# wg-perception/PartsBasedDetector

Measured on AMD Instinct MI355X. Metric: detect() frames/sec, 640x480, 26-part person model, higher is better.
Workload: dtype f32

## Files before the change

### partsbaseddetector_amd/csrc/k_conv_split32.hpp

```cpp
typedef __bf16 bf16x8 __attribute__((ext_vector_type(8)));
typedef _Float16 f16x8 __attribute__((ext_vector_type(8)));
typedef unsigned u32x4 __attribute__((ext_vector_type(4)));
typedef float f32x4 __attribute__((ext_vector_type(4)));
typedef float f32x16 __attribute__((ext_vector_type(16)));

template <int NT, int NW, int PIN, int NS = 3, bool MIX = false>
__global__ __launch_bounds__(64 * NW) __attribute__((amdgpu_waves_per_eu(1, PIN ? 1 : 2))) void k_conv_split32(const ConvTile* __restrict__ tiles, const LevelDev* __restrict__ levels,
                                                             const uint16_t* __restrict__ feat, const uint16_t* __restrict__ filt,
                                                             float* __restrict__ resp, int nf, int ntl_bank, int ntile0, int ngroups,
                                                             int ntiles_total, int kh, int kw, const float* __restrict__ oscale) {
  extern __shared__ __attribute__((aligned(16))) char smem[];
  constexpr int ROWS = 4 * NW, NHALVES = 16 / ROWS, NTHR = 64 * NW, PPC = 4 * NS;
  const int TW = 16 + kw - 1, TH = ROWS + kh - 1, NC = TW * TH, PLANE = NC * 64;
  const int R = NHALVES * ngroups;
  const int lin = blockIdx.x;
  const int grp = lin / (8 * R), rem = lin - grp * (8 * R);
  const int tile_i = grp * 8 + (rem & 7), role = rem >> 3;
  if (tile_i >= ntiles_total) return;
  const int half = role & (NHALVES - 1), ngroup = role / NHALVES;
  const ConvTile t = tiles[tile_i];
  const LevelDev lv = levels[t.level];
  const int H = lv.ch, W = lv.cw;
  const int ty0 = t.y0 + ROWS * half, tx0 = t.x0;
  if (ty0 >= H) return;
  const int tid = threadIdx.x, lane = tid & 63, wave = __builtin_amdgcn_readfirstlane(tid >> 6);
  const uint16_t* F = feat + lv.cell_off * (NS * PBD_FLEN);
  {
    const int NPC = NC * PPC, oy = ty0 - kh / 2, ox = tx0 - kw / 2;
    constexpr unsigned ONE = NS == 3 ? 0x3F800000u : 0x6C000000u;
    auto cell_of = [](int i) { return NS == 3 ? (int)(((unsigned)i * 43691u) >> 19) : i >> 3; };
    const unsigned magic_tw = 0xFFFFFFFFu / (unsigned)TW + 1u;
    constexpr int BATCH = 12;
    for (int i0 = 0; i0 < NPC; i0 += NTHR * BATCH) {
      u32x4 v[BATCH];
#pragma unroll
      for (int j = 0; j < BATCH; ++j) {
        const int i = min(i0 + j * NTHR + tid, NPC - 1);
        const int cell = cell_of(i), piece = i - cell * PPC;
        const int cy = (int)__umulhi((unsigned)cell, magic_tw), cx = cell - cy * TW;
        const int y = min(max(oy + cy, 0), H - 1), x = min(max(ox + cx, 0), W - 1);
        v[j] = *(const u32x4*)(F + ((size_t)(y * W + x) * (NS * PBD_FLEN) + piece * 8));
      }
#pragma unroll
      for (int j = 0; j < BATCH; ++j) {
        const int i = i0 + j * NTHR + tid;
        if (i < NPC) {
          const int cell = cell_of(i), piece = i - cell * PPC;
          const int cy = (int)__umulhi((unsigned)cell, magic_tw), cx = cell - cy * TW;
          const int y = oy + cy, x = ox + cx;
          const bool inside = y >= 0 && y < H && x >= 0 && x < W;
          const u32x4 border = u32x4{0u, 0u, 0u, piece == 3 ? ONE : 0u};
          const int q = piece & 3;
          *(u32x4*)(smem + (piece >> 2) * PLANE + cell * 64 + ((q ^ ((cell >> 2) & 3)) << 4)) = inside ? v[j] : border;
        }
      }
    }
  }
  __syncthreads();
  const int col = lane & 15, kb = lane >> 4;
  const bool inner = col >= 4 && col < 12;
  const int kk = inner ? col - 4 : col < 4 ? col : col - 8;
  const int pos = ((kk >> 1) << 2) + (inner ? 0 : 2) + (kk & 1);
  const int vw = min(16, W - tx0), vh = min(ROWS, H - ty0), ncell = vw * vh;
  const int nmt = (ncell + 15) >> 4;
  const int mvalid = __builtin_amdgcn_readfirstlane(max(0, min(4, (nmt - wave + NW - 1) / NW)));
  const unsigned vw_magic = 65535u / (unsigned)vw + 1u;
  int cl0[4], cofs[4];
  bool cval[4];
#pragma unroll
  for (int m = 0; m < 4; ++m) {
    const int idx = 16 * (wave + NW * m) + pos;
    cval[m] = idx < ncell;
    const int ic = min(idx, ncell - 1);
    const int cy = (int)(((unsigned)ic * vw_magic) >> 16), cx = ic - cy * vw;
    cl0[m] = cy * TW + cx;
    cofs[m] = (ty0 + cy) * W + tx0 + cx;
  }
  const int ntb = ntile0 + ngroup * NT;
  const size_t bs_split = (size_t)ntl_bank * 512, bs_kstep = NS * bs_split, bs_tap = 2 * bs_kstep;
  const uint16_t* bl = filt + (size_t)ntb * 512 + (size_t)(kb >> 1) * bs_kstep + (kb & 1) * 256 + col * 8;
#ifdef PBD_BANK_PRIO
  __builtin_amdgcn_s_setprio(PBD_BANK_PRIO);
#endif

  constexpr int NTRI = NS == 3 ? 2 : 1;
  auto mfma3 = [](int tri, f32x4& d, const u32x4 (&fb)[NS], const u32x4 (&fa)[NS]) __attribute__((always_inline)) {
    if constexpr (NS == 3) {
      if (tri == 0)
        asm volatile("v_mfma_f32_16x16x32_bf16 %0, %1, %2, %0\n\tv_mfma_f32_16x16x32_bf16 %0, %3, %4, %0\n\tv_mfma_f32_16x16x32_bf16 %0, %5, %6, %0"
                     : "+a"(d) : "v"(fb[1]), "v"(fa[1]), "v"(fb[2]), "v"(fa[0]), "v"(fb[0]), "v"(fa[2]));
      else
        asm volatile("v_mfma_f32_16x16x32_bf16 %0, %1, %2, %0\n\tv_mfma_f32_16x16x32_bf16 %0, %3, %4, %0\n\tv_mfma_f32_16x16x32_bf16 %0, %3, %2, %0"
                     : "+a"(d) : "v"(fb[1]), "v"(fa[0]), "v"(fb[0]), "v"(fa[1]));
    } else {
      asm volatile("v_mfma_f32_16x16x32_f16 %0, %1, %2, %0\n\tv_mfma_f32_16x16x32_f16 %0, %3, %4, %0\n\tv_mfma_f32_16x16x32_f16 %0, %3, %2, %0"
                   : "+a"(d) : "v"(fb[1]), "v"(fa[0]), "v"(fb[0]), "v"(fa[1]));
    }
  };

  auto k_loop = [&](auto mv_tag) __attribute__((always_inline)) {
    constexpr int MV = decltype(mv_tag)::value, NU = 2 * MV * NTRI, NLD = 2 * NS, LPT = (NLD + NU - 2) / (NU - 1);
    static_assert(NU >= 2 && LPT * (NU - 1) >= NLD, "a step's statements carry the next step's filter loads");
    u32x4 a[4][NS], b[2][2][NS];
    f32x4 acc[2 * NT][MV];
#pragma unroll
    for (int ft = 0; ft < 2 * NT; ++ft)
// ... 24 lines not shown
          for (int m = 0; m < MV; ++m) {
#pragma unroll
            for (int q = 0; q < NTRI; ++q) {
              const int u = (h * MV + m) * NTRI + q;
              mfma3(q + 2 - NTRI, acc[2 * nt + h][m], b[slot][h], a[m]);
              if (u * LPT < NLD) {
                __builtin_amdgcn_sched_barrier(0);
#pragma unroll
                for (int k = u * LPT; k < (u + 1) * LPT && k < NLD; ++k)
                  b[slot ^ 1][k / NS][k % NS] = *(const u32x4*)(pl + (k % NS) * bs_split + (k / NS) * 128);
                __builtin_amdgcn_sched_barrier(0);
              }
            }
            if (last && h == 1) {
              __builtin_amdgcn_sched_barrier(0);
              ld_a(m, nextofs);
              __builtin_amdgcn_sched_barrier(0);
            }
          }
      }
    };
    const int ntap = kh * kw;
#pragma unroll
    for (int k = 0; k < NLD; ++k) b[0][k / NS][k % NS] = *(const u32x4*)(bl + (k % NS) * bs_split + (k / NS) * 128);
#pragma unroll
    for (int m = 0; m < MV; ++m) ld_a(m, 0);
    pad_acc();
    int ti = 0, tj = 0;
    const uint16_t* pt = bl;
    auto one_tap = [&](auto p_tag, int tap) __attribute__((always_inline)) {
      if (++tj == kw) { tj = 0; ++ti; }
      const bool more = tap + 1 < ntap;
      const uint16_t* pn = more ? pt + bs_tap : pt;
      tap_body(p_tag, pt, pn, more ? ti * TW + tj : 0);
      pt = pn;
    };
#pragma unroll 1
    for (int tap = 0; tap < ntap; tap += 1 + (NT & 1)) {
      one_tap(std::integral_constant<int, 0>(), tap);
      if constexpr (NT & 1) {
        if (tap + 1 >= ntap) break;
        one_tap(std::integral_constant<int, 1>(), tap + 1);
      }
    }
    pad_acc();

    float* Rl = resp + lv.cell_off * nf;
    const size_t HW = (size_t)H * W;
    int nfw = nf;
    if constexpr (MIX) { Rl += (size_t)(t.pad & 0xFFFF) * HW; nfw = t.pad >> 16; }
#pragma unroll
    for (int m = 0; m < MV; ++m) {
      if (cval[m]) {
#pragma unroll
        for (int ft = 0; ft < 2 * NT; ++ft) {
          const int f0 = 32 * ntb + 16 * ft + 4 * kb;
          float* pl = Rl + (size_t)f0 * HW + cofs[m];
#pragma unroll
          for (int r = 0; r < 4; ++r)
            if (f0 + r < nfw) pl[(size_t)r * HW] = NS == 3 ? acc[ft][m][r] : acc[ft][m][r] * oscale[f0 + r];
        }
      }
    }
  };
  switch (mvalid) {
    case 4: k_loop(std::integral_constant<int, 4>()); break;
    case 3: k_loop(std::integral_constant<int, 3>()); break;
    case 2: k_loop(std::integral_constant<int, 2>()); break;
    case 1: k_loop(std::integral_constant<int, 1>()); break;
    default: return;
  }
}

template <int NT, int NW, int PIN, int NS = 3, bool MIX = false>
static void launch_conv_split_t(const ConvTile* tiles, int ntiles, const LevelDev* levels, const uint16_t* feat_split, const uint16_t* wS,
                                float* resp, int nf, int ntl_bank, int ntile0, int ngroups, int kh, int kw, hipStream_t s, const float* oscale = nullptr,
                                int nf_stride = 0) {
  constexpr int ROWS = 4 * NW, NHALVES = 16 / ROWS;
  const size_t lds = (size_t)(16 + kw - 1) * (ROWS + kh - 1) * 64 * NS;
  static LdsOptIn optin;
  optin.ensure((const void*)k_conv_split32<NT, NW, PIN, NS, MIX>, lds);
  const int grid = (ntiles + 7) / 8 * 8 * NHALVES * ngroups;
  hipLaunchKernelGGL((k_conv_split32<NT, NW, PIN, NS, MIX>), dim3(grid), dim3(64 * NW), lds, s, tiles, levels, feat_split, wS, resp, MIX ? nf_stride : nf,
                     ntl_bank, ntile0, ngroups, ntiles, kh, kw, oscale);
}
template <int NW, int PIN, int NS, bool MIX = false>
static void launch_conv_split_groups(const ConvTile* tiles, int ntiles, const LevelDev* levels, const uint16_t* feat_split, const uint16_t* wS,
                                     float* resp, int nf, int kh, int kw, const float* oscale, hipStream_t s, int nf_stride = 0, int G = 5) {
  const int ntl = conv_split_ntiles(nf), full = ntl / G, rest = ntl - G * full;
  auto go = [&](int nt, int ntile0, int ngroups) {
    switch (nt) {
      case 1: launch_conv_split_t<1, NW, PIN, NS, MIX>(tiles, ntiles, levels, feat_split, wS, resp, nf, ntl, ntile0, ngroups, kh, kw, s, oscale, nf_stride); break;
      case 2: launch_conv_split_t<2, NW, PIN, NS, MIX>(tiles, ntiles, levels, feat_split, wS, resp, nf, ntl, ntile0, ngroups, kh, kw, s, oscale, nf_stride); break;
      case 3: launch_conv_split_t<3, NW, PIN, NS, MIX>(tiles, ntiles, levels, feat_split, wS, resp, nf, ntl, ntile0, ngroups, kh, kw, s, oscale, nf_stride); break;
      case 4: launch_conv_split_t<4, NW, PIN, NS, MIX>(tiles, ntiles, levels, feat_split, wS, resp, nf, ntl, ntile0, ngroups, kh, kw, s, oscale, nf_stride); break;
      case 5: launch_conv_split_t<5, NW, PIN, NS, MIX>(tiles, ntiles, levels, feat_split, wS, resp, nf, ntl, ntile0, ngroups, kh, kw, s, oscale, nf_stride); break;
      default: break;
    }
  };
  if (full) go(G, 0, full);
  if (rest) go(rest, G * full, 1);
}
```

### partsbaseddetector_amd/csrc/k_pyramid.hip

```cpp
#include <algorithm>
#include "pbd_internal.hpp"

typedef __attribute__((aligned(1))) unsigned u32_unaligned;

__device__ __forceinline__ int sat_short_dev(float v) {
  int i = __float2int_rn(v);
  return i < -32768 ? -32768 : (i > 32767 ? 32767 : i);
}

#define RPX 4
__global__ __launch_bounds__(256) void k_resize_linear_u8(const PyrJob* __restrict__ jobs, int cn, int sstride,
                                                          const uint8_t* __restrict__ src0, uint8_t* __restrict__ pyr) {
  const PyrJob a = jobs[blockIdx.y];
  const int dw = a.dw, dh = a.dh, sw = a.sw, sh = a.sh;
  const uint8_t* src = src0 + a.soff;
  uint8_t* dst = pyr + a.doff;
  const bool copy = (dw == sw && dh == sh);
  if (copy) {
    const int rowb = dw * cn, wpr = (rowb + 3) >> 2, nw = wpr * dh;
    for (int i = blockIdx.x * blockDim.x + threadIdx.x; i < nw; i += gridDim.x * blockDim.x) {
      const int y = i / wpr, k = i - y * wpr;
      const uint8_t* s = src + (size_t)y * sstride + 4 * k;
      uint8_t* d = dst + (size_t)y * rowb + 4 * k;
      if (4 * k + 4 <= rowb) *(u32_unaligned*)d = *(const u32_unaligned*)s;
      else for (int b = 0; 4 * k + b < rowb; ++b) d[b] = s[b];
    }
    return;
  }
  const double scale_x = 1. / ((double)dw / sw), scale_y = 1. / ((double)dh / sh);
  const int gpr = (dw + RPX - 1) / RPX, ngrp = gpr * dh;
  for (int i = blockIdx.x * blockDim.x + threadIdx.x; i < ngrp; i += gridDim.x * blockDim.x) {
    const int dy = i / gpr, gx = i - dy * gpr;
    float fy = (float)((dy + 0.5) * scale_y - 0.5);
    int sy = (int)floorf(fy);
    fy -= sy;
    const int b0 = sat_short_dev((1.f - fy) * 2048), b1 = sat_short_dev(fy * 2048);
    const int sy0 = sy < 0 ? 0 : (sy >= sh ? sh - 1 : sy);
    const int sy1 = sy + 1 < 0 ? 0 : (sy + 1 >= sh ? sh - 1 : sy + 1);
    const uint8_t* R0 = src + (size_t)sy0 * sstride;
    const uint8_t* R1 = src + (size_t)sy1 * sstride;
    uint8_t ob[RPX * 3];
    const int npx = min(RPX, dw - gx * RPX);
#pragma unroll
    for (int p = 0; p < RPX; ++p) {
      const int dx = min(gx * RPX + p, dw - 1);
      float fx = (float)((dx + 0.5) * scale_x - 0.5);
      int sx = (int)floorf(fx);
      fx -= sx;
      if (sx < 0) { fx = 0; sx = 0; }
      const bool edge = (sx + 1 >= sw);
      if (sx >= sw - 1) { fx = 0; sx = sw - 1; }
      const int a0 = sat_short_dev((1.f - fx) * 2048), a1 = sat_short_dev(fx * 2048);
      const uint8_t* S0 = R0 + sx * cn;
      const uint8_t* S1 = R1 + sx * cn;
      uint8_t p0[6], p1[6];
      if (cn == 3 && !edge) {
        const unsigned w00 = *(const u32_unaligned*)S0, w01 = *(const unsigned short __attribute__((aligned(1)))*)(S0 + 4);
        const unsigned w10 = *(const u32_unaligned*)S1, w11 = *(const unsigned short __attribute__((aligned(1)))*)(S1 + 4);
#pragma unroll
        for (int b = 0; b < 4; ++b) { p0[b] = (uint8_t)(w00 >> (8 * b)); p1[b] = (uint8_t)(w10 >> (8 * b)); }
        p0[4] = (uint8_t)w01; p0[5] = (uint8_t)(w01 >> 8); p1[4] = (uint8_t)w11; p1[5] = (uint8_t)(w11 >> 8);
      } else {
#pragma unroll
        for (int b = 0; b < 6; ++b) {
          const int o = (b < cn || !edge) && b < 2 * cn ? b : 0;
          p0[b] = S0[o]; p1[b] = S1[o];
        }
      }
#pragma unroll
      for (int c = 0; c < 3; ++c) {
        if (c < cn) {
          int r0, r1;
          if (edge) { r0 = p0[c] * 2048; r1 = p1[c] * 2048; }
          else { r0 = p0[c] * a0 + p0[c + cn] * a1; r1 = p1[c] * a0 + p1[c + cn] * a1; }
          const int v = (((b0 * (r0 >> 4)) >> 16) + ((b1 * (r1 >> 4)) >> 16) + 2) >> 2;
          ob[p * 3 + c] = (uint8_t)(v < 0 ? 0 : (v > 255 ? 255 : v));
        }
      }
    }
    uint8_t* d = dst + ((size_t)dy * dw + gx * RPX) * cn;
    if (cn == 3 && npx == RPX) {
#pragma unroll
      for (int k = 0; k < 3; ++k)
        *(u32_unaligned*)(d + 4 * k) = (unsigned)ob[4 * k] | ((unsigned)ob[4 * k + 1] << 8) | ((unsigned)ob[4 * k + 2] << 16) | ((unsigned)ob[4 * k + 3] << 24);
    } else {
      for (int p = 0; p < npx; ++p)
        for (int c = 0; c < cn; ++c) d[p * cn + c] = ob[p * 3 + c];
    }
  }
}

__device__ __forceinline__ int reflect101_dev(int p, int len) {
  if (len == 1) return 0;
  while ((unsigned)p >= (unsigned)len) p = p < 0 ? -p : 2 * len - 2 - p;
  return p;
}

#define PD_TW 32
#define PD_TH 8
#define PD_SW (2 * PD_TW + 3)
#define PD_SH (2 * PD_TH + 3)
template <int CN>
__global__ __launch_bounds__(256) void k_pyrdown_u8(const PyrJob* __restrict__ jobs, uint8_t* __restrict__ pyr) {
  constexpr int cn = CN;
  __shared__ __attribute__((aligned(4))) uint8_t tile[PD_SH][(PD_SW * CN + 3) & ~3];
  __shared__ unsigned short hs[PD_SH][PD_TW * CN];
  const PyrJob a = jobs[blockIdx.z];
  const int sw = a.sw, sh = a.sh;
  const int dw = (sw + 1) / 2, dh = (sh + 1) / 2;
  const int x0 = blockIdx.x * PD_TW, y0 = blockIdx.y * PD_TH;
  if (x0 >= dw || y0 >= dh) return;
  const uint8_t* src = pyr + a.soff;
  uint8_t* dst = pyr + a.doff;
  const int tid = threadIdx.x;
  const int sx0 = 2 * x0 - 2, sy0 = 2 * y0 - 2;
  const int rowb = PD_SW * cn, srow = sw * cn;
  {
    const int wpr = (rowb + 3) >> 2, nw = wpr * PD_SH;
    const bool xin = sx0 >= 0 && sx0 + PD_SW <= sw;
    for (int i = tid; i < nw; i += 256) {
      const int r = i / wpr, k = i - r * wpr;
      const uint8_t* srow_p = src + (size_t)reflect101_dev(sy0 + r, sh) * srow;
      unsigned v;
      if (xin && sx0 * cn + 4 * k + 4 <= srow) {
        v = *(const u32_unaligned*)(srow_p + sx0 * cn + 4 * k);
      } else {
        v = 0;
#pragma unroll
        for (int b = 0; b < 4; ++b) {
          const int cb = 4 * k + b;
          const int px = cb / cn, ch = cb - px * cn;
          const int sx = reflect101_dev(sx0 + min(px, PD_SW - 1), sw);
          v |= (unsigned)srow_p[sx * cn + ch] << (8 * b);
        }
      }
      *(unsigned*)&tile[r][4 * k] = v;
    }
  }
  __syncthreads();
  {
    const int n = PD_SH * PD_TW * cn;
    for (int i = tid; i < n; i += 256) {
      const int r = i / (PD_TW * cn), xc = i - r * (PD_TW * cn);
      const int x = xc / cn, c = xc - x * cn;
      const uint8_t* p = &tile[r][2 * x * cn + c];
      hs[r][xc] = (unsigned short)(p[0] + 4 * p[cn] + 6 * p[2 * cn] + 4 * p[3 * cn] + p[4 * cn]);
    }
  }
  __syncthreads();
  {
    const int n = PD_TH * PD_TW * cn;
    for (int i = tid; i < n; i += 256) {
      const int y = i / (PD_TW * cn), xc = i - y * (PD_TW * cn);
      const int x = xc / cn;
      if (y0 + y < dh && x0 + x < dw) {
        const int s = hs[2 * y][xc] + 4 * hs[2 * y + 1][xc] + 6 * hs[2 * y + 2][xc] + 4 * hs[2 * y + 3][xc] + hs[2 * y + 4][xc];
        dst[((size_t)(y0 + y) * dw + x0) * cn + xc] = (uint8_t)((s + 128) >> 8);
      }
    }
  }
}

void launch_resize(const PyrJob* jobs, int njobs, int maxpix, int cn, int sstride, const uint8_t* src, uint8_t* pyr, hipStream_t s) {
  if (njobs <= 0) return;
  dim3 grid((maxpix / RPX + 255) / 256 + 1, njobs);
  hipLaunchKernelGGL(k_resize_linear_u8, grid, dim3(256), 0, s, jobs, cn, sstride, src, pyr);
}

void launch_pyrdown(const PyrJob* jobs, int njobs, int maxw, int maxh, int cn, uint8_t* pyr, hipStream_t s) {
  if (njobs <= 0) return;
  dim3 grid((maxw + PD_TW - 1) / PD_TW, (maxh + PD_TH - 1) / PD_TH, njobs);
  if (cn == 3) hipLaunchKernelGGL(k_pyrdown_u8<3>, grid, dim3(256), 0, s, jobs, pyr);
  else hipLaunchKernelGGL(k_pyrdown_u8<1>, grid, dim3(256), 0, s, jobs, pyr);
}

template <typename PT> struct PyrWork { typedef float type; };
template <> struct PyrWork<double> { typedef double type; };
template <typename PT> __device__ __forceinline__ PT pyr_cast(typename PyrWork<PT>::type v) { return (PT)v; }
template <> __device__ __forceinline__ uint16_t pyr_cast<uint16_t>(float v) {
  const int i = __float2int_rn(v);
  return (uint16_t)(i < 0 ? 0 : (i > 65535 ? 65535 : i));
}

template <typename PT>
__global__ __launch_bounds__(256) void k_resize_linear_any(const PyrJob* __restrict__ jobs, int cn, int sstride,
                                                           const uint8_t* __restrict__ src0, uint8_t* __restrict__ pyr) {
  typedef typename PyrWork<PT>::type WT;
  const PyrJob a = jobs[blockIdx.y];
  const int dw = a.dw, dh = a.dh, sw = a.sw, sh = a.sh;
  const PT* src = (const PT*)(src0 + a.soff);
  PT* dst = (PT*)(pyr + a.doff);
  const int n = dw * dh * cn;
  if (dw == sw && dh == sh) {
    for (int i = blockIdx.x * blockDim.x + threadIdx.x; i < n; i += gridDim.x * blockDim.x) {
      const int y = i / (dw * cn), xc = i - y * (dw * cn);
      dst[i] = src[(size_t)y * sstride + xc];
    }
    return;
  }
  const double scale_x = 1. / ((double)dw / sw), scale_y = 1. / ((double)dh / sh);
  for (int i = blockIdx.x * blockDim.x + threadIdx.x; i < n; i += gridDim.x * blockDim.x) {
    const int dy = i / (dw * cn), xc = i - dy * (dw * cn);
    const int dx = xc / cn, c = xc - dx * cn;
    float fy = (float)((dy + 0.5) * scale_y - 0.5);
    const int sy = (int)floorf(fy);
    fy -= sy;
    float fx = (float)((dx + 0.5) * scale_x - 0.5);
    int sx = (int)floorf(fx);
    fx -= sx;
    if (sx < 0) { fx = 0; sx = 0; }
    const bool edge = (sx + 1 >= sw);
    if (sx >= sw - 1) { fx = 0; sx = sw - 1; }
    const float a0 = 1.f - fx, a1 = fx;
    const WT b0 = 1.f - fy, b1 = fy;
    const int sy0 = sy < 0 ? 0 : (sy >= sh ? sh - 1 : sy);
    const int sy1 = sy + 1 < 0 ? 0 : (sy + 1 >= sh ? sh - 1 : sy + 1);
    const PT* S0 = src + (size_t)sy0 * sstride + sx * cn + c;
    const PT* S1 = src + (size_t)sy1 * sstride + sx * cn + c;
    WT r0, r1;
    if (edge) { r0 = (WT)(S0[0] * 1); r1 = (WT)(S1[0] * 1); }
    else { r0 = (WT)(S0[0] * a0 + S0[cn] * a1); r1 = (WT)(S1[0] * a0 + S1[cn] * a1); }
    dst[i] = pyr_cast<PT>(r0 * b0 + r1 * b1);
  }
}

template <typename PT>
// ... 48 lines not shown
```

Baseline: 2570.

## Restructure split-conv LDS staging row-wise with scalar row pointers and leaner epilogue stores

The feature tile staging loop now assigns each lane a fixed column and piece and walks rows, so per-element divisions and 2D clamps are computed once per lane. Row base addresses become wave-uniform scalar pointers, which reduces VALU address arithmetic before the barrier. The LDS swizzle is rewritten in an XOR form that must match the consumer's layout. The output epilogue hoists the base pointer, skips fully out-of-range filter blocks, uses scalar offsets, and loads the scale vector once in the unchecked path.

```diff
diff --git a/partsbaseddetector_amd/csrc/conv_split_stage.hpp b/partsbaseddetector_amd/csrc/conv_split_stage.hpp
--- /dev/null
+++ b/partsbaseddetector_amd/csrc/conv_split_stage.hpp
@@ -0,0 +1,33 @@
+#pragma once
+#ifdef __HIPCC__
+#define PBD_SS_HD __host__ __device__ __forceinline__
+#else
+#define PBD_SS_HD inline
+#endif
+
+struct SplitStageLane {
+  int cx, piece;
+  unsigned lds;
+  unsigned part;
+};
+template <int PPC>
+PBD_SS_HD SplitStageLane split_stage_lane(int p) {
+  SplitStageLane l;
+  l.cx = (int)((unsigned)p / (unsigned)PPC);
+  l.piece = p - l.cx * PPC;
+  l.lds = (unsigned)l.cx * 64u + ((unsigned)(l.piece & 3) << 4);
+  l.part = (unsigned)l.piece >> 2;
+  return l;
+}
+PBD_SS_HD unsigned split_stage_lds(unsigned rowofs, const SplitStageLane& l, unsigned plane_bytes) {
+  const unsigned t = rowofs + l.lds;
+  return (t ^ ((t >> 4) & 0x30u)) + l.part * plane_bytes;
+}
+PBD_SS_HD int split_stage_clamp(int first, int i, int n, bool* inside) {
+  const int c = first + i;
+  *inside = c >= 0 && c < n;
+  return c < 0 ? 0 : c > n - 1 ? n - 1 : c;
+}
+template <int PPC>
+PBD_SS_HD unsigned split_stage_src(int xc, const SplitStageLane& l) { return (unsigned)xc * (16u * PPC) + (unsigned)l.piece * 16u; }
+PBD_SS_HD int split_stage_passes(int tw, int ppc, int nthr) { return (tw * ppc + nthr - 1) / nthr; }
diff --git a/partsbaseddetector_amd/csrc/k_conv_split32.hpp b/partsbaseddetector_amd/csrc/k_conv_split32.hpp
--- a/partsbaseddetector_amd/csrc/k_conv_split32.hpp
+++ b/partsbaseddetector_amd/csrc/k_conv_split32.hpp
@@ -1,8 +1,18 @@
+#include "conv_split_stage.hpp"
 typedef __bf16 bf16x8 __attribute__((ext_vector_type(8)));
 typedef _Float16 f16x8 __attribute__((ext_vector_type(8)));
 typedef unsigned u32x4 __attribute__((ext_vector_type(4)));
 typedef float f32x4 __attribute__((ext_vector_type(4)));
 typedef float f32x16 __attribute__((ext_vector_type(16)));
+
+#define PBD_GLOBAL_AS __attribute__((address_space(1)))
+__device__ __forceinline__ unsigned long long uniform_u64(unsigned long long u) {
+  const unsigned lo = __builtin_amdgcn_readfirstlane((unsigned)u), hi = __builtin_amdgcn_readfirstlane((unsigned)(u >> 32));
+  unsigned long long s = ((unsigned long long)hi << 32) | lo;
+  asm("" : "+s"(s));
+  return s;
+}
+__device__ __forceinline__ PBD_GLOBAL_AS char* uniform_ptr(const void* p) { return (PBD_GLOBAL_AS char*)uniform_u64((unsigned long long)p); }
 
 template <int NT, int NW, int PIN, int NS = 3, bool MIX = false>
 __global__ __launch_bounds__(64 * NW) __attribute__((amdgpu_waves_per_eu(1, PIN ? 1 : 2))) void k_conv_split32(const ConvTile* __restrict__ tiles, const LevelDev* __restrict__ levels,
@@ -26,32 +36,41 @@
   const int tid = threadIdx.x, lane = tid & 63, wave = __builtin_amdgcn_readfirstlane(tid >> 6);
   const uint16_t* F = feat + lv.cell_off * (NS * PBD_FLEN);
   {
-    const int NPC = NC * PPC, oy = ty0 - kh / 2, ox = tx0 - kw / 2;
+    const int RP = TW * PPC, oy = ty0 - kh / 2, ox = tx0 - kw / 2;
     constexpr unsigned ONE = NS == 3 ? 0x3F800000u : 0x6C000000u;
-    auto cell_of = [](int i) { return NS == 3 ? (int)(((unsigned)i * 43691u) >> 19) : i >> 3; };
-    const unsigned magic_tw = 0xFFFFFFFFu / (unsigned)TW + 1u;
     constexpr int BATCH = 12;
-    for (int i0 = 0; i0 < NPC; i0 += NTHR * BATCH) {
-      u32x4 v[BATCH];
-#pragma unroll
-      for (int j = 0; j < BATCH; ++j) {
-        const int i = min(i0 + j * NTHR + tid, NPC - 1);
-        const int cell = cell_of(i), piece = i - cell * PPC;
-        const int cy = (int)__umulhi((unsigned)cell, magic_tw), cx = cell - cy * TW;
-        const int y = min(max(oy + cy, 0), H - 1), x = min(max(ox + cx, 0), W - 1);
-        v[j] = *(const u32x4*)(F + ((size_t)(y * W + x) * (NS * PBD_FLEN) + piece * 8));
-      }
-#pragma unroll
-      for (int j = 0; j < BATCH; ++j) {
-        const int i = i0 + j * NTHR + tid;
-        if (i < NPC) {
-          const int cell = cell_of(i), piece = i - cell * PPC;
-          const int cy = (int)__umulhi((unsigned)cell, magic_tw), cx = cell - cy * TW;
-          const int y = oy + cy, x = ox + cx;
-          const bool inside = y >= 0 && y < H && x >= 0 && x < W;
-          const u32x4 border = u32x4{0u, 0u, 0u, piece == 3 ? ONE : 0u};
-          const int q = piece & 3;
-          *(u32x4*)(smem + (piece >> 2) * PLANE + cell * 64 + ((q ^ ((cell >> 2) & 3)) << 4)) = inside ? v[j] : border;
+    const char* Fb = (const char*)F;
+    const size_t rowbytes = (size_t)W * (16 * PPC);
+#pragma unroll 1
+    for (int p0 = 64 * wave; p0 < RP; p0 += NTHR) {
+      const int p = p0 + lane;
+      const SplitStageLane sl = split_stage_lane<PPC>(min(p, RP - 1));
+      bool xin;
+      const int xc = split_stage_clamp(ox, sl.cx, W, &xin);
+      const unsigned src = split_stage_src<PPC>(xc, sl);
+      const unsigned bw3 = sl.piece == 3 ? ONE : 0u;
+#pragma unroll 1
+      for (int r0 = 0; r0 < TH; r0 += BATCH) {
+        u32x4 v[BATCH];
+#pragma unroll
+        for (int j = 0; j < BATCH; ++j) {
+          bool yin;
+          const int yc = split_stage_clamp(oy, min(r0 + j, TH - 1), H, &yin);
+          v[j] = *(const PBD_GLOBAL_AS u32x4*)(uniform_ptr(Fb + (size_t)yc * rowbytes) + src);
+        }
+        __builtin_amdgcn_sched_barrier(0);
+        if (p < RP) {
+#pragma unroll
+          for (int j = 0; j < BATCH; ++j) {
+            const int cy = r0 + j;
+            if (j == 0 || cy < TH) {
+              bool yin;
+              split_stage_clamp(oy, cy, H, &yin);
+              const bool inside = yin && xin;
+              const u32x4 border = u32x4{0u, 0u, 0u, bw3};
+              *(u32x4*)(smem + split_stage_lds((unsigned)(cy * TW) * 64u, sl, (unsigned)PLANE)) = inside ? v[j] : border;
+            }
+          }
         }
       }
     }
@@ -182,13 +201,23 @@
 #pragma unroll
     for (int m = 0; m < MV; ++m) {
       if (cval[m]) {
+        float* pm = Rl + ((size_t)(32 * ntb + 4 * kb) * HW + cofs[m]);
 #pragma unroll
         for (int ft = 0; ft < 2 * NT; ++ft) {
-          const int f0 = 32 * ntb + 16 * ft + 4 * kb;
-          float* pl = Rl + (size_t)f0 * HW + cofs[m];
-#pragma unroll
-          for (int r = 0; r < 4; ++r)
-            if (f0 + r < nfw) pl[(size_t)r * HW] = NS == 3 ? acc[ft][m][r] : acc[ft][m][r] * oscale[f0 + r];
+          const int fb = 32 * ntb + 16 * ft, f0 = fb + 4 * kb;
+          if (fb >= nfw) continue;
+          asm volatile("" : "+a"(acc[ft][m]));
+          auto store4 = [&](auto checked) __attribute__((always_inline)) {
+            constexpr bool CHECKED = decltype(checked)::value;
+            f32x4 os = f32x4{1.f, 1.f, 1.f, 1.f};
+            if constexpr (NS != 3 && !CHECKED) os = *(const f32x4*)(oscale + f0);
+#pragma unroll
+            for (int r = 0; r < 4; ++r)
+              if (!CHECKED || f0 + r < nfw)
+                *(float*)((char*)pm + uniform_u64((size_t)(16 * ft + r) * HW * 4)) = NS == 3 ? acc[ft][m][r] : acc[ft][m][r] * (CHECKED ? oscale[f0 + r] : os[r]);
+          };
+          if (fb + 16 <= nfw) store4(std::false_type());
+          else store4(std::true_type());
         }
       }
     }
diff --git a/profiles/split_bank_staging/count_valu.py b/profiles/split_bank_staging/count_valu.py
--- /dev/null
+++ b/profiles/split_bank_staging/count_valu.py
@@ -0,0 +1,56 @@
+import re
+import sys
+
+
+def kernel_lines(text, nt, ns, mix):
+    name = "_Z14k_conv_split32ILi%dELi4ELi2ELi%dELb%dEE" % (nt, ns, mix)
+    m = re.search(r"^%s\w*:.*\n" % name, text, re.M)
+    end = text.index(".end_amdhsa_kernel", m.end())
+    return [l.strip() for l in text[m.end():end].split("\n")]
+
+
+def is_valu(l):
+    return l.startswith("v_") and not l.startswith("v_mfma")
+
+
+def main():
+    path = sys.argv[1]
+    nt, ns, mix = (int(a) for a in sys.argv[2:5]) if len(sys.argv) >= 5 else (5, 3, 0)
+    ls = kernel_lines(open(path).read(), nt, ns, mix)
+    bar = next(i for i, l in enumerate(ls) if l.startswith("s_barrier"))
+    pre = ls[:bar]
+    out = {"before_barrier": sum(map(is_valu, pre))}
+    loops, cur = {}, None
+    for l in pre:
+        m = re.match(r"^\.LBB(\d+_\d+):\s*;\s*(.*)$", l)
+        if m:
+            own, note = m.group(1), m.group(2)
+            h = re.search(r"in Loop: Header=BB(\d+_\d+) Depth=(\d+)", note)
+            cur = (own if "Loop Header" in note or "Parent Loop" in note else None) or (h.group(1) if h else None)
+        elif re.match(r"^\.LBB\d+_\d+:", l):
+            cur = None
+        elif cur:
+            c = loops.setdefault(cur, [0, 0, 0])
+            c[0] += is_valu(l); c[1] += l.startswith("global_load"); c[2] += l.startswith("ds_write")
+    for h, c in loops.items():
+        out["loop_BB%s_valu/loads/ds_writes" % h] = "%d / %d / %d" % tuple(c)
+    top = 32 * nt - 1
+    hits = [i for i, l in enumerate(ls) if re.search(r"\ba%d\b" % top, l) and not l.startswith("v_mfma") and "s_nop" not in l and i > bar]
+    if hits:
+        lo = hi = hits[-1]
+        while lo > bar and not ls[lo].startswith("v_mfma"):
+            lo -= 1
+        while hi < len(ls) - 1 and not ls[hi].startswith("v_mfma"):
+            hi += 1
+        seg = ls[lo + 1:hi]
+        out["epilogue_mv4_stretch"] = sum(map(is_valu, seg))
+        out["epilogue_mv4_stores"] = sum(l.startswith("global_store") for l in seg)
+        out["epilogue_mv4_accvgpr_reads"] = sum(l.startswith("v_accvgpr_read") for l in seg)
+    out["kernel_valu_static"] = sum(map(is_valu, ls))
+    out["kernel_mfma_static"] = sum(l.startswith("v_mfma") for l in ls)
+    for k, v in out.items():
+        print("%-40s %s" % (k, v))
+
+
+if __name__ == "__main__":
+    main()
```

Measured after the change: 2588 (median of 6 runs). About the same (+0.7%).

## Restructure pyramid resize and pyrDown kernels around packed SIMD byte math

Applied to the files above, without the earlier changes.

Rewrites the linear resize kernel so each wave walks a band of rows, with per-column coefficients hoisted and row coefficients broadcast via readlane. The interpolation uses udot2 and perm packed-u16 arithmetic, and the copy path uses 16-byte vector copies. The pyrDown kernel now stages word-sized rows, computes horizontal and vertical 5-tap sums on packed u16 pairs, and writes 4-byte outputs. The intent is to cut integer ALU work, index division and narrow byte stores in the pyramid build, at the cost of much more intricate code whose rounding must still match the old results.

```diff
diff --git a/partsbaseddetector_amd/csrc/k_pyramid.hip b/partsbaseddetector_amd/csrc/k_pyramid.hip
--- a/partsbaseddetector_amd/csrc/k_pyramid.hip
+++ b/partsbaseddetector_amd/csrc/k_pyramid.hip
@@ -1,110 +1,114 @@
 #include <algorithm>
 #include "pbd_internal.hpp"
+#include "pyr_core.hpp"
 
 typedef __attribute__((aligned(1))) unsigned u32_unaligned;
-
-__device__ __forceinline__ int sat_short_dev(float v) {
-  int i = __float2int_rn(v);
-  return i < -32768 ? -32768 : (i > 32767 ? 32767 : i);
-}
-
-#define RPX 4
-__global__ __launch_bounds__(256) void k_resize_linear_u8(const PyrJob* __restrict__ jobs, int cn, int sstride,
-                                                          const uint8_t* __restrict__ src0, uint8_t* __restrict__ pyr) {
+typedef __attribute__((aligned(1))) unsigned short u16_unaligned;
+typedef unsigned u32x4 __attribute__((ext_vector_type(4)));
+typedef __attribute__((aligned(1))) u32x4 u32x4_unaligned;
+__device__ __forceinline__ int lane_to_scalar(int v, int lane) { return __builtin_amdgcn_readlane(v, lane); }
+
+__device__ __forceinline__ unsigned lane_offset(unsigned v) { asm volatile("" : "+v"(v)); return v; }
+
+template <int CN, bool WIDE>
+__device__ __forceinline__ void rz_band(int strip, int band, int lane, int wave, const uint8_t* __restrict__ src, int sstride,
+                                        uint8_t* __restrict__ dst, int sw, int sh, int dw, int dh, double scale_x, double scale_y) {
+  const int x0 = rz_group(strip, lane) * RZ_RPX, rowb = dw * CN;
+  RzCol col[RZ_RPX];
+#pragma unroll
+  for (int p = 0; p < RZ_RPX; ++p) {
+    if (WIDE) col[p] = rz_col(min(x0 + p, dw - 1), scale_x, sw, CN);
+    else { col[p].off = 0; col[p].w = 2048u << 4; }
+  }
+  int vy0, vy1, vb0, vb1;
+  rz_coef_y(min(rz_row(band, wave, lane & (RZ_RPW - 1)), dh - 1), scale_y, sh, &vy0, &vy1, &vb0, &vb1);
+  const int nk = rz_nrows(band, wave, dh);
+  const int npx = min(RZ_RPX, dw - x0);
+  for (int k = 0; k < nk; ++k) {
+    const int sy0 = lane_to_scalar(vy0, k), sy1 = lane_to_scalar(vy1, k);
+    const unsigned bw0 = (unsigned)lane_to_scalar(vb0, k) << 16, bw1 = (unsigned)lane_to_scalar(vb1, k) << 16;
+    const uint8_t* R0 = src + (size_t)sy0 * sstride;
+    const uint8_t* R1 = src + (size_t)sy1 * sstride;
+    uint8_t* D = dst + (size_t)rz_row(band, wave, k) * rowb;
+    if (npx <= 0) continue;
+    unsigned t0[RZ_RPX * CN], t1[RZ_RPX * CN];
+#pragma unroll
+    for (int p = 0; p < RZ_RPX; ++p) {
+      unsigned P0[CN], P1[CN];
+      if constexpr (!WIDE) {
+#pragma unroll
+        for (int c = 0; c < CN; ++c) { P0[c] = (unsigned)R0[c] << 8; P1[c] = (unsigned)R1[c] << 8; }
+      } else if constexpr (CN == 3) {
+        const unsigned o = lane_offset((unsigned)col[p].off);
+        const unsigned w00 = *(const u32_unaligned*)(R0 + o), w01 = *(const u16_unaligned*)(R0 + o + 4);
+        const unsigned w10 = *(const u32_unaligned*)(R1 + o), w11 = *(const u16_unaligned*)(R1 + o + 4);
+        rz_gather<CN>(w00, w01, P0); rz_gather<CN>(w10, w11, P1);
+      } else {
+        const unsigned o = lane_offset((unsigned)col[p].off);
+        const unsigned w0 = *(const u16_unaligned*)(R0 + o), w1 = *(const u16_unaligned*)(R1 + o);
+        rz_gather<CN>(w0, 0u, P0); rz_gather<CN>(w1, 0u, P1);
+      }
+      rz_pixel<CN>(P0, P1, col[p].w, bw0, bw1, t0 + p * CN, t1 + p * CN);
+    }
+    unsigned ow[CN];
+#pragma unroll
+    for (int j = 0; j < CN; ++j) ow[j] = rz_pack4(t0 + 4 * j, t1 + 4 * j);
+    uint8_t* d = D + lane_offset((unsigned)PYR_MUL24(x0, CN));
+    if (npx == RZ_RPX) {
+#pragma unroll
+      for (int j = 0; j < CN; ++j) *(u32_unaligned*)(d + 4 * j) = ow[j];
+    } else {
+#pragma unroll
+      for (int j = 0; j < CN; ++j)
+#pragma unroll
+        for (int i = 0; i < 4; ++i)
+          if (4 * j + i < npx * CN) d[4 * j + i] = (uint8_t)(ow[j] >> (8 * i));
+    }
+  }
+}
+
+template <int CN>
+__global__ __launch_bounds__(RZ_SG * RZ_WAVES) void k_resize_linear_u8(const PyrJob* __restrict__ jobs, int sstride,
+                                                                       const uint8_t* __restrict__ src0, uint8_t* __restrict__ pyr) {
   const PyrJob a = jobs[blockIdx.y];
   const int dw = a.dw, dh = a.dh, sw = a.sw, sh = a.sh;
   const uint8_t* src = src0 + a.soff;
   uint8_t* dst = pyr + a.doff;
+  const int lane = rz_lane(threadIdx.x), wave = __builtin_amdgcn_readfirstlane(rz_wave(threadIdx.x));
+  const int rowb = dw * CN;
   const bool copy = (dw == sw && dh == sh);
+  const int nstrips = rz_strips(copy ? rz_copy_groups(rowb) : rz_groups(dw)), nbands = rz_bands(dh);
+  int strip = blockIdx.x, band = 0;
+  rz_walk(&strip, &band, nstrips);
   if (copy) {
-    const int rowb = dw * cn, wpr = (rowb + 3) >> 2, nw = wpr * dh;
-    for (int i = blockIdx.x * blockDim.x + threadIdx.x; i < nw; i += gridDim.x * blockDim.x) {
-      const int y = i / wpr, k = i - y * wpr;
-      const uint8_t* s = src + (size_t)y * sstride + 4 * k;
-      uint8_t* d = dst + (size_t)y * rowb + 4 * k;
-      if (4 * k + 4 <= rowb) *(u32_unaligned*)d = *(const u32_unaligned*)s;
-      else for (int b = 0; 4 * k + b < rowb; ++b) d[b] = s[b];
+    for (; band < nbands; strip += gridDim.x, rz_walk(&strip, &band, nstrips)) {
+      const int b = rz_group(strip, lane) * RZ_CPB, nk = rz_nrows(band, wave, dh);
+      if (b >= rowb) continue;
+      for (int k = 0; k < nk; ++k) {
+        const int y = rz_row(band, wave, k);
+        const unsigned bo = lane_offset((unsigned)b);
+        const uint8_t* s = src + (size_t)y * sstride + bo;
+        uint8_t* d = dst + (size_t)y * rowb + bo;
+        if (b + RZ_CPB <= rowb) *(u32x4_unaligned*)d = *(const u32x4_unaligned*)s;
+        else for (int i = 0; b + i < rowb; ++i) d[i] = s[i];
+      }
     }
     return;
   }
-  const double scale_x = 1. / ((double)dw / sw), scale_y = 1. / ((double)dh / sh);
-  const int gpr = (dw + RPX - 1) / RPX, ngrp = gpr * dh;
-  for (int i = blockIdx.x * blockDim.x + threadIdx.x; i < ngrp; i += gridDim.x * blockDim.x) {
-    const int dy = i / gpr, gx = i - dy * gpr;
-    float fy = (float)((dy + 0.5) * scale_y - 0.5);
-    int sy = (int)floorf(fy);
-    fy -= sy;
-    const int b0 = sat_short_dev((1.f - fy) * 2048), b1 = sat_short_dev(fy * 2048);
-    const int sy0 = sy < 0 ? 0 : (sy >= sh ? sh - 1 : sy);
-    const int sy1 = sy + 1 < 0 ? 0 : (sy + 1 >= sh ? sh - 1 : sy + 1);
-    const uint8_t* R0 = src + (size_t)sy0 * sstride;
-    const uint8_t* R1 = src + (size_t)sy1 * sstride;
-    uint8_t ob[RPX * 3];
-    const int npx = min(RPX, dw - gx * RPX);
-#pragma unroll
-    for (int p = 0; p < RPX; ++p) {
-      const int dx = min(gx * RPX + p, dw - 1);
-      float fx = (float)((dx + 0.5) * scale_x - 0.5);
-      int sx = (int)floorf(fx);
-      fx -= sx;
-      if (sx < 0) { fx = 0; sx = 0; }
-      const bool edge = (sx + 1 >= sw);
-      if (sx >= sw - 1) { fx = 0; sx = sw - 1; }
-      const int a0 = sat_short_dev((1.f - fx) * 2048), a1 = sat_short_dev(fx * 2048);
-      const uint8_t* S0 = R0 + sx * cn;
-      const uint8_t* S1 = R1 + sx * cn;
-      uint8_t p0[6], p1[6];
-      if (cn == 3 && !edge) {
-        const unsigned w00 = *(const u32_unaligned*)S0, w01 = *(const unsigned short __attribute__((aligned(1)))*)(S0 + 4);
-        const unsigned w10 = *(const u32_unaligned*)S1, w11 = *(const unsigned short __attribute__((aligned(1)))*)(S1 + 4);
-#pragma unroll
-        for (int b = 0; b < 4; ++b) { p0[b] = (uint8_t)(w00 >> (8 * b)); p1[b] = (uint8_t)(w10 >> (8 * b)); }
-        p0[4] = (uint8_t)w01; p0[5] = (uint8_t)(w01 >> 8); p1[4] = (uint8_t)w11; p1[5] = (uint8_t)(w11 >> 8);
-      } else {
-#pragma unroll
-        for (int b = 0; b < 6; ++b) {
-          const int o = (b < cn || !edge) && b < 2 * cn ? b : 0;
-          p0[b] = S0[o]; p1[b] = S1[o];
-        }
-      }
-#pragma unroll
-      for (int c = 0; c < 3; ++c) {
-        if (c < cn) {
-          int r0, r1;
-          if (edge) { r0 = p0[c] * 2048; r1 = p1[c] * 2048; }
-          else { r0 = p0[c] * a0 + p0[c + cn] * a1; r1 = p1[c] * a0 + p1[c + cn] * a1; }
-          const int v = (((b0 * (r0 >> 4)) >> 16) + ((b1 * (r1 >> 4)) >> 16) + 2) >> 2;
-          ob[p * 3 + c] = (uint8_t)(v < 0 ? 0 : (v > 255 ? 255 : v));
-        }
-      }
-    }
-    uint8_t* d = dst + ((size_t)dy * dw + gx * RPX) * cn;
-    if (cn == 3 && npx == RPX) {
-#pragma unroll
-      for (int k = 0; k < 3; ++k)
-        *(u32_unaligned*)(d + 4 * k) = (unsigned)ob[4 * k] | ((unsigned)ob[4 * k + 1] << 8) | ((unsigned)ob[4 * k + 2] << 16) | ((unsigned)ob[4 * k + 3] << 24);
-    } else {
-      for (int p = 0; p < npx; ++p)
-        for (int c = 0; c < cn; ++c) d[p * cn + c] = ob[p * 3 + c];
-    }
-  }
-}
-
-__device__ __forceinline__ int reflect101_dev(int p, int len) {
-  if (len == 1) return 0;
-  while ((unsigned)p >= (unsigned)len) p = p < 0 ? -p : 2 * len - 2 - p;
-  return p;
-}
-
-#define PD_TW 32
-#define PD_TH 8
-#define PD_SW (2 * PD_TW + 3)
-#define PD_SH (2 * PD_TH + 3)
+  const double scale_x = rz_scale(dw, sw), scale_y = rz_scale(dh, sh);
+  for (; band < nbands; strip += gridDim.x, rz_walk(&strip, &band, nstrips)) {
+    if (sw >= 2) rz_band<CN, true>(strip, band, lane, wave, src, sstride, dst, sw, sh, dw, dh, scale_x, scale_y);
+    else rz_band<CN, false>(strip, band, lane, wave, src, sstride, dst, sw, sh, dw, dh, scale_x, scale_y);
+  }
+}
+
+__device__ __forceinline__ int reflect101_dev(int p, int len) { return pd_reflect101(p, len); }
+
 template <int CN>
-__global__ __launch_bounds__(256) void k_pyrdown_u8(const PyrJob* __restrict__ jobs, uint8_t* __restrict__ pyr) {
-  constexpr int cn = CN;
-  __shared__ __attribute__((aligned(4))) uint8_t tile[PD_SH][(PD_SW * CN + 3) & ~3];
-  __shared__ unsigned short hs[PD_SH][PD_TW * CN];
+__global__ __launch_bounds__(PD_THREADS) void k_pyrdown_u8(const PyrJob* __restrict__ jobs, uint8_t* __restrict__ pyr) {
+  typedef PdGeo<CN> G;
+  __shared__ __attribute__((aligned(8))) unsigned tile[PD_SH][G::wpr];
+  __shared__ __attribute__((aligned(8))) unsigned hs[PD_SH][G::hsw];
   const PyrJob a = jobs[blockIdx.z];
   const int sw = a.sw, sh = a.sh;
   const int dw = (sw + 1) / 2, dh = (sh + 1) / 2;
@@ -114,64 +118,82 @@
   uint8_t* dst = pyr + a.doff;
   const int tid = threadIdx.x;
   const int sx0 = 2 * x0 - 2, sy0 = 2 * y0 - 2;
-  const int rowb = PD_SW * cn, srow = sw * cn;
+  const int srow = sw * CN;
+  const bool small = (size_t)sh * srow < ((size_t)1 << 24);
   {
-    const int wpr = (rowb + 3) >> 2, nw = wpr * PD_SH;
-    const bool xin = sx0 >= 0 && sx0 + PD_SW <= sw;
-    for (int i = tid; i < nw; i += 256) {
-      const int r = i / wpr, k = i - r * wpr;
-      const uint8_t* srow_p = src + (size_t)reflect101_dev(sy0 + r, sh) * srow;
-      unsigned v;
-      if (xin && sx0 * cn + 4 * k + 4 <= srow) {
-        v = *(const u32_unaligned*)(srow_p + sx0 * cn + 4 * k);
-      } else {
-        v = 0;
-#pragma unroll
-        for (int b = 0; b < 4; ++b) {
-          const int cb = 4 * k + b;
-          const int px = cb / cn, ch = cb - px * cn;
-          const int sx = reflect101_dev(sx0 + min(px, PD_SW - 1), sw);
-          v |= (unsigned)srow_p[sx * cn + ch] << (8 * b);
+    const int k = pd_stage_word<CN>(tid);
+    if (k < G::wpr) {
+      const bool inside = pd_word_inside<CN>(k, sx0, srow);
+      const int cb = sx0 * CN + 4 * k;
+#pragma unroll
+      for (int i = 0; i < (PD_SH + G::rps - 1) / G::rps; ++i) {
+        const int r = G::lpr == 64 ? __builtin_amdgcn_readfirstlane(pd_stage_row<CN>(tid, i)) : pd_stage_row<CN>(tid, i);
+        if (r >= PD_SH) break;
+        const int ry = pd_reflect101(sy0 + r, sh);
+        const uint8_t* srow_p = src + (small ? (size_t)__umul24(ry, srow) : (size_t)ry * srow);
+        unsigned v;
+        if (inside) {
+          v = *(const u32_unaligned*)(srow_p + lane_offset((unsigned)cb));
+        } else {
+          v = 0;
+#pragma unroll
+          for (int b = 0; b < 4; ++b) v |= (unsigned)srow_p[pd_src_byte<CN>(4 * k + b, sx0, sw)] << (8 * b);
         }
-      }
-      *(unsigned*)&tile[r][4 * k] = v;
+        tile[r][k] = v;
+      }
     }
   }
   __syncthreads();
   {
-    const int n = PD_SH * PD_TW * cn;
-    for (int i = tid; i < n; i += 256) {
-      const int r = i / (PD_TW * cn), xc = i - r * (PD_TW * cn);
-      const int x = xc / cn, c = xc - x * cn;
-      const uint8_t* p = &tile[r][2 * x * cn + c];
-      hs[r][xc] = (unsigned short)(p[0] + 4 * p[cn] + 6 * p[2 * cn] + 4 * p[3 * cn] + p[4 * cn]);
+    const int m = pd_h_item(tid);
+#pragma unroll
+    for (int pass = 0; pass < (PD_SH * PD_HITEMS + PD_THREADS - 1) / PD_THREADS; ++pass) {
+      const int r = pd_h_row(tid, pass);
+      if (r >= PD_SH) break;
+      unsigned W[G::hiw];
+#pragma unroll
+      for (int i = 0; i < G::hiw; ++i) W[i] = tile[r][pd_h_word<CN>(m) + i];
+      unsigned S[G::how];
+      pd_h_sums<CN>(W, S);
+#pragma unroll
+      for (int q = 0; q < G::how; ++q) hs[r][G::how * m + q] = S[q];
     }
   }
   __syncthreads();
   {
-    const int n = PD_TH * PD_TW * cn;
-    for (int i = tid; i < n; i += 256) {
-      const int y = i / (PD_TW * cn), xc = i - y * (PD_TW * cn);
-      const int x = xc / cn;
-      if (y0 + y < dh && x0 + x < dw) {
-        const int s = hs[2 * y][xc] + 4 * hs[2 * y + 1][xc] + 6 * hs[2 * y + 2][xc] + 4 * hs[2 * y + 3][xc] + hs[2 * y + 4][xc];
-        dst[((size_t)(y0 + y) * dw + x0) * cn + xc] = (uint8_t)((s + 128) >> 8);
-      }
+    const int k = pd_v_word(tid), y = pd_v_row(tid);
+    if (k < G::vwr && y0 + y < dh) {
+      unsigned lo[5], hi[5];
+#pragma unroll
+      for (int j = 0; j < 5; ++j) {
+        const uint2 v = *(const uint2*)&hs[2 * y + j][2 * k];
+        lo[j] = v.x; hi[j] = v.y;
+      }
+      const unsigned w = pd_v_bytes(lo, hi);
+      const int drow = dw * CN, bx = x0 * CN + 4 * k;
+      const int ye = __builtin_amdgcn_readfirstlane(y & ~1);
+      uint8_t* d = dst + (size_t)(y0 + ye) * drow + ((y & 1) ? drow : 0) + bx;
+      if (bx + 4 <= drow) *(u32_unaligned*)d = w;
+      else
+#pragma unroll
+        for (int b = 0; b < 4; ++b)
+          if (bx + b < drow) d[b] = (uint8_t)(w >> (8 * b));
     }
   }
 }
 
 void launch_resize(const PyrJob* jobs, int njobs, int maxpix, int cn, int sstride, const uint8_t* src, uint8_t* pyr, hipStream_t s) {
   if (njobs <= 0) return;
-  dim3 grid((maxpix / RPX + 255) / 256 + 1, njobs);
-  hipLaunchKernelGGL(k_resize_linear_u8, grid, dim3(256), 0, s, jobs, cn, sstride, src, pyr);
+  dim3 grid(rz_grid_x(maxpix), njobs);
+  if (cn == 3) hipLaunchKernelGGL(k_resize_linear_u8<3>, grid, dim3(RZ_SG * RZ_WAVES), 0, s, jobs, sstride, src, pyr);
+  else hipLaunchKernelGGL(k_resize_linear_u8<1>, grid, dim3(RZ_SG * RZ_WAVES), 0, s, jobs, sstride, src, pyr);
 }
 
 void launch_pyrdown(const PyrJob* jobs, int njobs, int maxw, int maxh, int cn, uint8_t* pyr, hipStream_t s) {
   if (njobs <= 0) return;
   dim3 grid((maxw + PD_TW - 1) / PD_TW, (maxh + PD_TH - 1) / PD_TH, njobs);
-  if (cn == 3) hipLaunchKernelGGL(k_pyrdown_u8<3>, grid, dim3(256), 0, s, jobs, pyr);
-  else hipLaunchKernelGGL(k_pyrdown_u8<1>, grid, dim3(256), 0, s, jobs, pyr);
+  if (cn == 3) hipLaunchKernelGGL(k_pyrdown_u8<3>, grid, dim3(PD_THREADS), 0, s, jobs, pyr);
+  else hipLaunchKernelGGL(k_pyrdown_u8<1>, grid, dim3(PD_THREADS), 0, s, jobs, pyr);
 }
 
 template <typename PT> struct PyrWork { typedef float type; };
diff --git a/partsbaseddetector_amd/csrc/pyr_core.hpp b/partsbaseddetector_amd/csrc/pyr_core.hpp
--- /dev/null
+++ b/partsbaseddetector_amd/csrc/pyr_core.hpp
@@ -0,0 +1,190 @@
+#pragma once
+#include <math.h>
+#include <stdint.h>
+
+#ifdef __HIPCC__
+#define PYR_HD __host__ __device__ __forceinline__
+#else
+#define PYR_HD static inline
+#endif
+#ifdef __HIP_DEVICE_COMPILE__
+#define PYR_MUL24(a, b) __mul24((a), (b))
+PYR_HD int pyr_round(float v) { return __float2int_rn(v); }
+#else
+#define PYR_MUL24(a, b) ((a) * (b))
+PYR_HD int pyr_round(float v) { return (int)lrintf(v); }
+#endif
+
+#ifdef __clang__
+typedef unsigned short pyr_u16x2 __attribute__((ext_vector_type(2)));
+#else
+struct pyr_u16x2 { unsigned short x, y; };
+PYR_HD pyr_u16x2 operator+(pyr_u16x2 a, pyr_u16x2 b) { return pyr_u16x2{(unsigned short)(a.x + b.x), (unsigned short)(a.y + b.y)}; }
+PYR_HD pyr_u16x2 operator+(pyr_u16x2 a, unsigned short b) { return pyr_u16x2{(unsigned short)(a.x + b), (unsigned short)(a.y + b)}; }
+PYR_HD pyr_u16x2 operator*(pyr_u16x2 a, unsigned short b) { return pyr_u16x2{(unsigned short)(a.x * b), (unsigned short)(a.y * b)}; }
+PYR_HD pyr_u16x2 operator>>(pyr_u16x2 a, unsigned short b) { return pyr_u16x2{(unsigned short)(a.x >> b), (unsigned short)(a.y >> b)}; }
+#endif
+#ifdef __HIP_DEVICE_COMPILE__
+PYR_HD pyr_u16x2 pyr_lanes(unsigned v) { return __builtin_bit_cast(pyr_u16x2, v); }
+PYR_HD unsigned pyr_word(pyr_u16x2 v) { return __builtin_bit_cast(unsigned, v); }
+PYR_HD unsigned pyr_dot2(unsigned a, unsigned b, unsigned c) { return __builtin_amdgcn_udot2(pyr_lanes(a), pyr_lanes(b), c, false); }
+PYR_HD unsigned pyr_perm(unsigned hi, unsigned lo, unsigned sel) { return __builtin_amdgcn_perm(hi, lo, sel); }
+#else
+PYR_HD pyr_u16x2 pyr_lanes(unsigned v) { pyr_u16x2 r; r.x = (unsigned short)v; r.y = (unsigned short)(v >> 16); return r; }
+PYR_HD unsigned pyr_word(pyr_u16x2 v) { return (unsigned)v.x | ((unsigned)v.y << 16); }
+PYR_HD unsigned pyr_dot2(unsigned a, unsigned b, unsigned c) { return (a & 0xffffu) * (b & 0xffffu) + (a >> 16) * (b >> 16) + c; }
+PYR_HD unsigned pyr_perm(unsigned hi, unsigned lo, unsigned sel) {
+  const unsigned long long src = ((unsigned long long)hi << 32) | lo;
+  unsigned r = 0;
+  for (int i = 0; i < 4; ++i) {
+    const unsigned s = (sel >> (8 * i)) & 0xffu;
+    r |= (s < 8 ? (unsigned)(src >> (8 * s)) & 0xffu : 0u) << (8 * i);
+  }
+  return r;
+}
+#endif
+
+PYR_HD int pyr_sat_short(float v) {
+  const int i = pyr_round(v);
+  return i < -32768 ? -32768 : (i > 32767 ? 32767 : i);
+}
+
+#define RZ_RPX 4
+#define RZ_CPB 16
+#define RZ_SG 64
+#define RZ_WAVES 4
+#define RZ_RPW 8
+#define RZ_BH (RZ_WAVES * RZ_RPW)
+
+PYR_HD double rz_scale(int d, int s) { return 1. / ((double)d / s); }
+
+PYR_HD bool rz_coef_x(int dx, double scale_x, int sw, int* sx_, int* a0, int* a1) {
+  float fx = (float)((dx + 0.5) * scale_x - 0.5);
+  int sx = (int)floorf(fx);
+  fx -= sx;
+  if (sx < 0) { fx = 0; sx = 0; }
+  const bool edge = (sx + 1 >= sw);
+  if (sx >= sw - 1) { fx = 0; sx = sw - 1; }
+  *a0 = pyr_sat_short((1.f - fx) * 2048); *a1 = pyr_sat_short(fx * 2048);
+  *sx_ = sx;
+  return edge;
+}
+PYR_HD void rz_coef_y(int dy, double scale_y, int sh, int* sy0, int* sy1, int* b0, int* b1) {
+  float fy = (float)((dy + 0.5) * scale_y - 0.5);
+  const int sy = (int)floorf(fy);
+  fy -= sy;
+  *b0 = pyr_sat_short((1.f - fy) * 2048); *b1 = pyr_sat_short(fy * 2048);
+  *sy0 = sy < 0 ? 0 : (sy >= sh ? sh - 1 : sy);
+  *sy1 = sy + 1 < 0 ? 0 : (sy + 1 >= sh ? sh - 1 : sy + 1);
+}
+struct RzCol { int off; unsigned w; };
+PYR_HD RzCol rz_col(int dx, double scale_x, int sw, int cn) {
+  int sx, a0, a1;
+  const bool edge = rz_coef_x(dx, scale_x, sw, &sx, &a0, &a1);
+  RzCol c;
+  c.off = PYR_MUL24(edge ? sx - 1 : sx, cn);
+  c.w = edge ? (unsigned)a0 << 20 : ((unsigned)a0 << 4) | ((unsigned)a1 << 20);
+  return c;
+}
+
+template <int CN> PYR_HD void rz_gather(unsigned w_lo, unsigned w_hi, unsigned* P) {
+  if constexpr (CN == 3) {
+    P[0] = pyr_perm(w_hi, w_lo, 0x030c000cu);
+    P[1] = pyr_perm(w_hi, w_lo, 0x040c010cu);
+    P[2] = pyr_perm(w_hi, w_lo, 0x050c020cu);
+  } else {
+    P[0] = pyr_perm(0u, w_lo, 0x010c000cu);
+  }
+}
+template <int CN> PYR_HD void rz_pixel(const unsigned* P0, const unsigned* P1, unsigned cw, unsigned bw0, unsigned bw1, unsigned* t0, unsigned* t1) {
+  for (int c = 0; c < CN; ++c) {
+    t0[c] = pyr_dot2(pyr_dot2(P0[c], cw, 0u), bw0, 2u << 16);
+    t1[c] = pyr_dot2(pyr_dot2(P1[c], cw, 0u), bw1, 0u);
+  }
+}
+PYR_HD unsigned rz_pack4(const unsigned* t0, const unsigned* t1) {
+  const pyr_u16x2 lo = (pyr_lanes(pyr_perm(t0[1], t0[0], 0x07060302u)) + pyr_lanes(pyr_perm(t1[1], t1[0], 0x07060302u))) >> (unsigned short)2;
+  const pyr_u16x2 hi = (pyr_lanes(pyr_perm(t0[3], t0[2], 0x07060302u)) + pyr_lanes(pyr_perm(t1[3], t1[2], 0x07060302u))) >> (unsigned short)2;
+  return pyr_perm(pyr_word(hi), pyr_word(lo), 0x06040200u);
+}
+
+PYR_HD int rz_groups(int dw) { return (dw + RZ_RPX - 1) / RZ_RPX; }
+PYR_HD int rz_copy_groups(int rowb) { return (rowb + RZ_CPB - 1) / RZ_CPB; }
+PYR_HD int rz_strips(int ngroups) { return (ngroups + RZ_SG - 1) / RZ_SG; }
+PYR_HD int rz_bands(int dh) { return (dh + RZ_BH - 1) / RZ_BH; }
+PYR_HD void rz_walk(int* strip, int* band, int nstrips) {
+  while (*strip >= nstrips) { *strip -= nstrips; ++*band; }
+}
+PYR_HD int rz_lane(int tid) { return tid & (RZ_SG - 1); }
+PYR_HD int rz_wave(int tid) { return tid / RZ_SG; }
+PYR_HD int rz_group(int strip, int lane) { return strip * RZ_SG + lane; }
+PYR_HD int rz_row(int band, int wave, int k) { return band * RZ_BH + wave + RZ_WAVES * k; }
+PYR_HD int rz_nrows(int band, int wave, int dh) {
+  const int left = dh - band * RZ_BH - wave;
+  if (left <= 0) return 0;
+  const int n = (left + RZ_WAVES - 1) / RZ_WAVES;
+  return n < RZ_RPW ? n : RZ_RPW;
+}
+PYR_HD int rz_grid_x(int maxpix) { return maxpix / (RZ_RPX * RZ_SG * RZ_BH) + 8; }
+
+#define PD_TW 32
+#define PD_TH 8
+#define PD_SW (2 * PD_TW + 3)
+#define PD_SH (2 * PD_TH + 3)
+#define PD_THREADS 256
+#define PD_HITEMS 16
+
+PYR_HD int pd_reflect101(int p, int len) {
+  if (len == 1) return 0;
+  while ((unsigned)p >= (unsigned)len) p = p < 0 ? -p : 2 * len - 2 - p;
+  return p;
+}
+PYR_HD int pd_div3(int n) { return PYR_MUL24(n, 171) >> 9; }
+
+template <int CN> struct PdGeo {
+  static constexpr int rowb = PD_SW * CN;
+  static constexpr int wpr = (rowb + 3) / 4;
+  static constexpr int lpr = wpr > 32 ? 64 : 32;
+  static constexpr int rps = PD_THREADS / lpr;
+  static constexpr int hsw = PD_TW * CN / 2;
+  static constexpr int hiw = 2 * CN;
+  static constexpr int how = CN;
+  static constexpr int vwr = PD_TW * CN / 4;
+  static constexpr int vlr = 32;
+};
+template <int CN> PYR_HD int pd_stage_word(int tid) { return tid & (PdGeo<CN>::lpr - 1); }
+template <int CN> PYR_HD int pd_stage_row(int tid, int i) { return tid / PdGeo<CN>::lpr + i * PdGeo<CN>::rps; }
+template <int CN> PYR_HD int pd_src_byte(int cb, int sx0, int sw) {
+  const int px = CN == 3 ? pd_div3(cb) : cb, ch = cb - px * CN;
+  return PYR_MUL24(pd_reflect101(sx0 + (px < PD_SW - 1 ? px : PD_SW - 1), sw), CN) + ch;
+}
+template <int CN> PYR_HD bool pd_word_inside(int k, int sx0, int srow) {
+  const int b = PYR_MUL24(sx0, CN) + 4 * k;
+  return b >= 0 && b + 4 <= srow;
+}
+PYR_HD int pd_h_item(int tid) { return tid & (PD_HITEMS - 1); }
+PYR_HD int pd_h_row(int tid, int pass) { return tid / PD_HITEMS + pass * (PD_THREADS / PD_HITEMS); }
+template <int CN> PYR_HD int pd_h_word(int m) { return CN * m; }
+template <int CN> constexpr int pd_h_lo(int q) { return CN == 3 ? (q == 0 ? 0 : q == 1 ? 2 : 7) : 0; }
+template <int CN> constexpr int pd_h_hi(int q) { return CN == 3 ? (q == 0 ? 1 : q == 1 ? 6 : 8) : 2; }
+PYR_HD int pd_v_word(int tid) { return tid & 31; }
+PYR_HD int pd_v_row(int tid) { return tid / 32; }
+
+PYR_HD pyr_u16x2 pd_sum5(const pyr_u16x2* t) { return (t[0] + t[4]) + (t[1] + t[3]) * (unsigned short)4 + t[2] * (unsigned short)6; }
+template <int CN> PYR_HD void pd_h_sums(const unsigned* W, unsigned* out) {
+  for (int q = 0; q < PdGeo<CN>::how; ++q) {
+    pyr_u16x2 tap[5];
+    for (int j = 0; j < 5; ++j) {
+      const int bl = pd_h_lo<CN>(q) + j * CN, bh = pd_h_hi<CN>(q) + j * CN;
+      const int wl = bl >> 2, wh = bh >> 2;
+      tap[j] = pyr_lanes(pyr_perm(W[wh], W[wl], 0x0c000c00u | (unsigned)(bl & 3) | ((unsigned)((wh - wl) * 4 + (bh & 3)) << 16)));
+    }
+    out[q] = pyr_word(pd_sum5(tap));
+  }
+}
+PYR_HD unsigned pd_v_bytes(const unsigned* lo, const unsigned* hi) {
+  pyr_u16x2 a[5], b[5];
+  for (int j = 0; j < 5; ++j) { a[j] = pyr_lanes(lo[j]); b[j] = pyr_lanes(hi[j]); }
+  const pyr_u16x2 sa = (pd_sum5(a) + (unsigned short)128) >> (unsigned short)8, sb = (pd_sum5(b) + (unsigned short)128) >> (unsigned short)8;
+  return pyr_perm(pyr_word(sb), pyr_word(sa), 0x06040200u);
+}
```

Measured after the change: 2545 before, 2569 after, median of 6. About the same (+0.9%).
